# BadgerTechnologies/navigation

Hardware: AMD Instinct MI355X
Metric: scored trajectories/sec (whole node) + costmap inflation cells/sec, 400x400 map (higher is better)
Workload: dtype f64

## Files before the change

navigation_amd/csrc/planner_bfs_rows.hip:

```cpp
#include "planner_bfs_common.h"

namespace navgpu {

#ifdef NAVGPU_BFS_STATS
__device__ unsigned long long g_bfs_stats[16];
#define BFS_STAMP(v) const unsigned long long v = __builtin_amdgcn_s_memtime()
#define BFS_ACC(i, x) bst[i] += (x)
#else
#define BFS_STAMP(v)
#define BFS_ACC(i, x)
#endif
#ifndef NAVGPU_ROWS_RECORD_PAD
#define NAVGPU_ROWS_RECORD_PAD 4
#endif
constexpr uint32_t kRowsRecordPad = NAVGPU_ROWS_RECORD_PAD;
template <int W>
__host__ __device__ inline size_t bfs_rows_lds_words(uint32_t nx, uint32_t ny) {
  constexpr uint32_t Wp = (W + 3) & ~3u;
  const uint32_t nw = bfs_rows_waves(ny);
  return (((size_t)nw * kRowsPerWave * ((nx + 31) >> 5) + 3) & ~(size_t)3) + (size_t)kCareRows * kCareWords + (size_t)(nw + 2) * 2 * kRowsHalo * (2 * Wp + kRowsRecordPad);
}
__device__ __forceinline__ void rowsGroup4(const int g, const uint32_t aw, uint32_t& nz, uint32_t& lo, uint32_t& hi, uint32_t* __restrict__ b,
                                           uint32_t* __restrict__ f, const uint32_t L, const uint32_t R, uint32_t& p) {
  uint32_t u0, u1, u2, u3, t0, t1, t2, t3, st;
  uint64_t c0, c1, c2;
#define NAVGPU_ROWS_DPP " row_mask:0xf bank_mask:0xf bound_ctrl:1\n\t"
  asm volatile(
      "v_mov_b32 %[p], %[f3]\n\t"
      "s_bitcmp1_b32 %[aw], %[g]\n\t"
      "s_cbranch_scc0 1f\n\t"
      "v_alignbit_b32 %[u0], %[f0], %[L], 31\n\t"
      "v_alignbit_b32 %[u1], %[f1], %[f0], 31\n\t"
      "v_alignbit_b32 %[u2], %[f2], %[f1], 31\n\t"
      "v_alignbit_b32 %[u3], %[f3], %[f2], 31\n\t"
      "v_alignbit_b32 %[t0], %[f1], %[f0], 1\n\t"
      "v_alignbit_b32 %[t1], %[f2], %[f1], 1\n\t"
      "v_alignbit_b32 %[t2], %[f3], %[f2], 1\n\t"
      "v_alignbit_b32 %[t3], %[R], %[f3], 1\n\t"
      "v_or_b32_dpp %[u0], %[f0], %[u0] wave_shr:1" NAVGPU_ROWS_DPP
      "v_or_b32_dpp %[u1], %[f1], %[u1] wave_shr:1" NAVGPU_ROWS_DPP
      "v_or_b32_dpp %[u2], %[f2], %[u2] wave_shr:1" NAVGPU_ROWS_DPP
      "v_or_b32_dpp %[u3], %[f3], %[u3] wave_shr:1" NAVGPU_ROWS_DPP
      "v_or_b32_dpp %[t0], %[f0], %[t0] wave_shl:1" NAVGPU_ROWS_DPP
      "v_or_b32_dpp %[t1], %[f1], %[t1] wave_shl:1" NAVGPU_ROWS_DPP
      "v_or_b32_dpp %[t2], %[f2], %[t2] wave_shl:1" NAVGPU_ROWS_DPP
      "v_or_b32_dpp %[t3], %[f3], %[t3] wave_shl:1" NAVGPU_ROWS_DPP
      "v_bitop3_b32 %[f0], %[u0], %[b0], %[t0] bitop3:0x32\n\t"
      "v_bitop3_b32 %[f1], %[u1], %[b1], %[t1] bitop3:0x32\n\t"
      "v_bitop3_b32 %[f2], %[u2], %[b2], %[t2] bitop3:0x32\n\t"
      "v_bitop3_b32 %[f3], %[u3], %[b3], %[t3] bitop3:0x32\n\t"
      "v_or3_b32 %[b0], %[b0], %[u0], %[t0]\n\t"
      "v_or3_b32 %[b1], %[b1], %[u1], %[t1]\n\t"
      "v_or3_b32 %[b2], %[b2], %[u2], %[t2]\n\t"
      "v_or3_b32 %[b3], %[b3], %[u3], %[t3]\n\t"
      "v_or3_b32 %[u0], %[f0], %[f1], %[f2]\n\t"
      "v_cmp_ne_u32_e64 %[c1], 0, %[f0]\n\t"
      "v_or_b32_e32 %[u0], %[u0], %[f3]\n\t"
      "v_cmp_ne_u32_e64 %[c2], 0, %[f3]\n\t"
      "v_cmp_ne_u32_e64 %[c0], 0, %[u0]\n\t"
      "s_cmp_lg_u64 %[c1], 0\n\t"
      "s_cselect_b32 %[st], %[bit], 0\n\t"
      "s_or_b32 %[lo], %[lo], %[st]\n\t"
      "s_cmp_lg_u64 %[c2], 0\n\t"
      "s_cselect_b32 %[st], %[bit], 0\n\t"
      "s_or_b32 %[hi], %[hi], %[st]\n\t"
      "s_cmp_lg_u64 %[c0], 0\n\t"
      "s_cselect_b32 %[st], %[bit], 0\n\t"
      "s_or_b32 %[nz], %[nz], %[st]\n\t"
      "1:\n\t"
      : [b0] "+v"(b[0]), [b1] "+v"(b[1]), [b2] "+v"(b[2]), [b3] "+v"(b[3]), [f0] "+v"(f[0]), [f1] "+v"(f[1]), [f2] "+v"(f[2]), [f3] "+v"(f[3]),
        [p] "=&v"(p), [u0] "=&v"(u0), [u1] "=&v"(u1), [u2] "=&v"(u2), [u3] "=&v"(u3), [t0] "=&v"(t0), [t1] "=&v"(t1), [t2] "=&v"(t2),
        [t3] "=&v"(t3), [nz] "+s"(nz), [lo] "+s"(lo), [hi] "+s"(hi), [c0] "=&s"(c0), [c1] "=&s"(c1), [c2] "=&s"(c2), [st] "=&s"(st)
      : [aw] "s"(aw), [g] "n"(g), [bit] "n"(1 << g), [L] "v"(L), [R] "v"(R)
      : "scc");
#undef NAVGPU_ROWS_DPP
}
template <int W>
__device__ __forceinline__ void bfsRowsGrid(const PlannerDev& pl, const uint32_t inst, const int which, const uint32_t item) {
  constexpr int NG = (W + 3) / 4;
  constexpr int WP = NG * 4;
  constexpr int D = kRowsHalo;
  const BfsRegion rg = bfsRegion(pl, inst);
  const int bx0 = rg.x0, bx1 = rg.x1, by0 = rg.y0, by1 = rg.y1, care_ok = rg.care_ok;
  extern __shared__ __align__(16) uint32_t sm[];
  __shared__ uint32_t s_wave[16];
  __shared__ uint32_t s_flag[3];
  __shared__ uint32_t s_open[3];
  uint32_t tid_ = threadIdx.x, nx_ = pl.nx, ny_ = pl.ny;
  asm volatile("" : "+v"(tid_), "+s"(nx_), "+s"(ny_));
  const uint32_t tid = tid_;
  bfsStamp(pl, tid, item, 0);
  const Geom g = geomOf(pl, inst);
  const uint32_t nx = nx_, ny = ny_, Wr = (nx + 31) >> 5;
  const uint32_t nw = blockDim.x >> 6;
  const uint32_t lane = tid & 63u, wave_id = tid >> 6;
  const int row_i = (int)(wave_id * kRowsPerWave + lane) - D;
  const bool real = row_i >= 0 && row_i < (int)ny;
  const bool owner = real && lane >= (uint32_t)D && lane < 64u - D;
  const uint32_t row = real ? (uint32_t)row_i : 0u;
// ... 27 lines not shown

  uint32_t blocked[WP], fr[WP];
#pragma unroll
  for (int j = 0; j < WP; ++j) {
    blocked[j] = 0xFFFFFFFFu;
    fr[j] = 0;
    if (real && (uint32_t)j < Wr) {
      fr[j] = seedm[row * Wr + j];
      blocked[j] = ~(freew[row * Wr + j] & ((uint32_t)j + 1 == Wr ? last_mask : 0xFFFFFFFFu)) | fr[j];
    }
  }
  const bool wave_in_box = (int)(wave_id * kRowsPerWave) <= by1 && (int)((wave_id + 1) * kRowsPerWave) > by0;
  const bool row_in_box = owner && row_i >= by0 && row_i <= by1;
  const int w0 = rg.w0, w1 = rg.w1;
  const uint32_t region_groups = bfsRegionGroups(rg);
  uint32_t* drow = dist + (size_t)row * nx;
  auto storeCells = [&](int j, uint32_t cells, uint32_t value) { bfsStoreCells(drow + j * 32, cells, value, aligned4); };
  const bool pub_top = lane >= (uint32_t)D && lane < 2u * D, pub_bot = lane >= 64u - 2 * D && lane < 64u - D;
  const uint32_t pub_wr = (((wave_id + 1) * 2 + (pub_top ? 0u : 1u)) * D + (pub_top ? lane - D : lane - (64u - 2 * D))) * RS;
  const bool halo_top = lane < (uint32_t)D, halo_bot = lane >= 64u - D;
  const uint32_t halo_rd = ((halo_top ? (wave_id * 2 + 1) : ((wave_id + 2) * 2)) * D + (halo_top ? lane : lane - (64u - D))) * RS;
  constexpr uint32_t gmask = (1u << NG) - 1u;

  auto activity = [&]() -> uint32_t {
    uint32_t nz = 0, lo = 0, hi = 0;
#pragma unroll
    for (int q = 0; q < NG; ++q) {
      const uint32_t t = fr[4 * q] | fr[4 * q + 1] | fr[4 * q + 2] | fr[4 * q + 3];
      if (__builtin_amdgcn_ballot_w64(t != 0) != 0) {
        nz |= 1u << q;
        if (__builtin_amdgcn_ballot_w64(fr[4 * q] != 0) != 0) lo |= 1u << q;
        if (__builtin_amdgcn_ballot_w64(fr[4 * q + 3] != 0) != 0) hi |= 1u << q;
      }
    }
    return (nz | (lo >> 1) | (hi << 1)) & gmask;
  };
  if (wave_in_box) {
#pragma unroll
    for (int j = 0; j < W; ++j)
      if (j >= w0 && j <= w1 && row_in_box) storeCells(j, fr[j], 0u);
  }
  uint32_t a_own = activity();
  uint32_t level = 0, xch = 0, any_blk = 0;
  bfsStamp(pl, tid, item, 2);
  bool done = false;
#ifdef NAVGPU_BFS_STATS
  unsigned long long bst[9] = {0, 0, 0, 0, 0, 0, 0, 0, 0};
#endif
  while (!done) {
    for (int k = 0; k < D; ++k) {
      BFS_STAMP(ts1);
      BFS_ACC(5, 1);
      const uint32_t aw = __builtin_amdgcn_readfirstlane(a_own);
      BFS_ACC(7, aw != 0 ? 1 : 0);
      BFS_ACC(8, __builtin_popcount(aw));
      if (aw != 0) {
        uint32_t nz = 0, lo = 0, hi = 0;
        uint32_t p[2];
        const uint32_t zero = 0;
#pragma unroll
        for (int q = 0; q < NG; ++q)
          rowsGroup4(q, aw, nz, lo, hi, &blocked[4 * q], &fr[4 * q], q > 0 ? p[(q + 1) & 1] : zero, q + 1 < NG ? fr[q + 1 < NG ? 4 * q + 4 : 0] : zero,
                     p[q & 1]);
        BFS_STAMP(ts2);
        BFS_ACC(1, ts2 - ts1);
        if (wave_in_box && (nz & region_groups) != 0) {
#pragma unroll
          for (int q = 0; q < NG; ++q) {
            if (((nz & region_groups) >> q) & 1u) {
#pragma unroll
              for (int c = 0; c < 4; ++c) {
                const int j = 4 * q + c;
                if (j < W && j >= w0 && j <= w1) {
#ifndef NAVGPU_BFS_X_NOSTORE
                  if (row_in_box && fr[j < W ? j : 0] != 0) storeCells(j, fr[j < W ? j : 0], level + 1);
#endif
                }
              }
            }
          }
        }
        BFS_STAMP(ts3);
        BFS_ACC(2, ts3 - ts2);
        any_blk |= nz;
        a_own = (nz | (lo >> 1) | (hi << 1)) & gmask;
      }
      ++level;
    }
    BFS_STAMP(ts4);
    const uint32_t slot = xch % 3u;
    if (pub_top || pub_bot) {
#pragma unroll
      for (int q = 0; q < WP; q += 4) {
        *reinterpret_cast<uint4*>(edge + pub_wr + q) = make_uint4(fr[q], fr[q + 1], fr[q + 2], fr[q + 3]);
        *reinterpret_cast<uint4*>(edge + pub_wr + WP + q) = make_uint4(blocked[q], blocked[q + 1], blocked[q + 2], blocked[q + 3]);
      }
    }
    if (any_blk) s_flag[slot] = 1;
    if (wave_in_box) {
      uint32_t open_any = 0;
      const uint32_t rr = (uint32_t)(row_i - by0);
#pragma unroll
      for (int j = 0; j < W; ++j) {
        if (j >= w0 && j <= w1) {
          const uint32_t cw_i = (uint32_t)(j - w0);
          if (row_in_box) {
            const uint32_t care = (care_ok != 0 && cw_i < (uint32_t)kCareWords && rr < (uint32_t)kCareRows) ? care_l[rr * kCareWords + cw_i] : (care_ok ? 0u : 0xFFFFFFFFu);
            const int c_lo = max(bx0 - j * 32, 0), c_hi = min(bx1 - j * 32, 31);
            const uint32_t open = (~blocked[j] & care) | fr[j];
            if (c_hi >= c_lo) open_any |= open & (0xFFFFFFFFu >> (31 - c_hi)) & (0xFFFFFFFFu << c_lo);
          }
        }
      }
      if (open_any != 0) s_open[slot] = 1;
    }
    if (tid == 0) {
      s_flag[(xch + 1) % 3u] = 0;
      s_open[(xch + 1) % 3u] = 0;
    }
    BFS_STAMP(ts5);
    BFS_ACC(3, ts5 - ts4);
    __syncthreads();
    done = !s_flag[slot] || !s_open[slot];
    if (!done) {
      if ((halo_top || halo_bot) && real) {
#pragma unroll
        for (int q = 0; q < WP; q += 4) {
          const uint4 v = *reinterpret_cast<const uint4*>(edge + halo_rd + q);
          const uint4 b = *reinterpret_cast<const uint4*>(edge + halo_rd + WP + q);
          fr[q] = v.x;
          fr[q + 1] = v.y;
          fr[q + 2] = v.z;
          fr[q + 3] = v.w;
          blocked[q] = b.x;
          blocked[q + 1] = b.y;
          blocked[q + 2] = b.z;
          blocked[q + 3] = b.w;
        }
      }
      a_own = activity();
      __syncthreads();
    }
    ++xch;
    any_blk = 0;
    BFS_STAMP(ts6);
    BFS_ACC(4, ts6 - ts5);
  }
#ifdef NAVGPU_BFS_STATS
  if (lane == 0)
    for (int k = 0; k < 9; ++k) atomicAdd(&g_bfs_stats[k], bst[k]);
#endif
  bfsStamp(pl, tid, item, 3);

  __syncthreads();
  {
    uint32_t ex[WP], fb[WP];
#pragma unroll
    for (int j = 0; j < WP; ++j) {
      const bool in = owner && (uint32_t)j < Wr;
      fb[j] = in ? (freew[row * Wr + j] & ((uint32_t)j + 1 == Wr ? last_mask : 0xFFFFFFFFu)) : 0u;
      ex[j] = in ? ((blocked[j] & fb[j]) | seedm[row * Wr + j]) : 0u;
    }
    if (pub_top || pub_bot) {
#pragma unroll
      for (int j = 0; j < WP; ++j) edge[pub_wr + j] = ex[j];
    }
    __syncthreads();
// ... 24 lines not shown
__global__ __launch_bounds__(1024, 6) void k_bfs_rows(PlannerDev pl, uint32_t first, uint32_t count, uint32_t* next_item, const uint32_t* order) {
  __shared__ uint32_t s_item;
  const uint32_t total = count * pl.bfs_grids;
  for (;;) {
    if (threadIdx.x == 0) s_item = atomicAdd(next_item, 1u);
    __syncthreads();
    const uint32_t slot = s_item;
    if (slot >= total) break;
    const uint32_t item = order ? order[slot] : slot;
    const uint32_t g = item / count;
    bfsRowsGrid<W>(pl, first + (item - g * count), (int)pl.bfs_grids - 1 - (int)g, item);
    __syncthreads();
  }
}
constexpr int kRows2HaloLanes = 4;
constexpr int kRows2Levels = 2 * kRows2HaloLanes;
constexpr int kRows2PerWave = 2 * (64 - 2 * kRows2HaloLanes);
constexpr int kRows2Words = 32;
__host__ __device__ inline uint32_t bfs_rows2_waves(uint32_t ny) { return (ny + kRows2PerWave - 1) / kRows2PerWave; }
__host__ __device__ inline size_t bfs_rows2_lds_words(uint32_t ny) {
  return (size_t)kCareRows * kCareWords + (size_t)(bfs_rows2_waves(ny) + 2) * 2 * kRows2HaloLanes * 4 * kRows2Words;
}
template <int G>
__device__ __forceinline__ void rows2Group(const uint32_t aw, uint32_t& nz, uint32_t& lo, uint32_t& hi, uint32_t* __restrict__ bA, uint32_t* __restrict__ bB,
                                           uint32_t* __restrict__ fA, uint32_t* __restrict__ fB, uint32_t& pA, uint32_t& pB, const uint32_t rA,
                                           const uint32_t rB) {
  uint32_t u0, u1, u2, u3, v0, v1, v2, v3, h0, h1, h2, h3, st;
#define NAVGPU_ROWS2_HEAD_FIRST                \
  "s_bitcmp1_b32 %[aw], %[g]\n\t"              \
  "s_cbranch_scc0 1f\n\t"                      \
  "v_lshlrev_b32 %[u0], 1, %[fA0]\n\t"         \
  "v_lshlrev_b32 %[v0], 1, %[fB0]\n\t"
#define NAVGPU_ROWS2_HEAD_NEXT                 \
  "s_bitcmp1_b32 %[aw], %[g]\n\t"              \
  "s_cbranch_scc0 1f\n\t"                      \
  "s_bitcmp1_b32 %[aw], %[gp]\n\t"             \
  "s_cbranch_scc1 3f\n\t"                      \
  "v_lshlrev_b32 %[u0], 1, %[fA0]\n\t"         \
  "v_lshlrev_b32 %[v0], 1, %[fB0]\n\t"         \
  "s_branch 4f\n\t"                            \
  "3:\n\t"                                     \
  "v_alignbit_b32 %[u0], %[fA0], %[pA], 31\n\t" \
  "v_alignbit_b32 %[v0], %[fB0], %[pB], 31\n\t" \
  "4:\n\t"
#define NAVGPU_ROWS2_BODY(HEAD)                                                                        \
  asm volatile(                                                                                        \
      HEAD                                                                                             \
      "v_alignbit_b32 %[u1], %[fA1], %[fA0], 31\n\t"                                                   \
      "v_alignbit_b32 %[u2], %[fA2], %[fA1], 31\n\t"                                                   \
      "v_alignbit_b32 %[u3], %[fA3], %[fA2], 31\n\t"                                                   \
// ... 22 lines not shown
      "v_or_b32_dpp %[v1], %[fA1], %[v1] wave_shl:1 row_mask:0xf bank_mask:0xf bound_ctrl:1\n\t"       \
      "v_or_b32_dpp %[v2], %[fA2], %[v2] wave_shl:1 row_mask:0xf bank_mask:0xf bound_ctrl:1\n\t"       \
      "v_or_b32_dpp %[v3], %[fA3], %[v3] wave_shl:1 row_mask:0xf bank_mask:0xf bound_ctrl:1\n\t"       \
      "v_or3_b32 %[v0], %[v0], %[h0], %[fA0]\n\t"                                                      \
      "v_or3_b32 %[v1], %[v1], %[h1], %[fA1]\n\t"                                                      \
      "v_or3_b32 %[v2], %[v2], %[h2], %[fA2]\n\t"                                                      \
      "v_or3_b32 %[v3], %[v3], %[h3], %[fA3]\n\t"                                                      \
      "v_bitop3_b32 %[fA0], %[u0], %[bA0], %[u0] bitop3:0x30\n\t"                                      \
      "v_bitop3_b32 %[fA1], %[u1], %[bA1], %[u1] bitop3:0x30\n\t"                                      \
      "v_bitop3_b32 %[fA2], %[u2], %[bA2], %[u2] bitop3:0x30\n\t"                                      \
      "v_bitop3_b32 %[fA3], %[u3], %[bA3], %[u3] bitop3:0x30\n\t"                                      \
      "v_bitop3_b32 %[fB0], %[v0], %[bB0], %[v0] bitop3:0x30\n\t"                                      \
      "v_bitop3_b32 %[fB1], %[v1], %[bB1], %[v1] bitop3:0x30\n\t"                                      \
      "v_bitop3_b32 %[fB2], %[v2], %[bB2], %[v2] bitop3:0x30\n\t"                                      \
      "v_bitop3_b32 %[fB3], %[v3], %[bB3], %[v3] bitop3:0x30\n\t"                                      \
      "v_or_b32_e32 %[bA0], %[bA0], %[u0]\n\t"                                                         \
      "v_or_b32_e32 %[bA1], %[bA1], %[u1]\n\t"                                                         \
      "v_or_b32_e32 %[bA2], %[bA2], %[u2]\n\t"                                                         \
      "v_or_b32_e32 %[bA3], %[bA3], %[u3]\n\t"                                                         \
      "v_or_b32_e32 %[bB0], %[bB0], %[v0]\n\t"                                                         \
      "v_or_b32_e32 %[bB1], %[bB1], %[v1]\n\t"                                                         \
      "v_or_b32_e32 %[bB2], %[bB2], %[v2]\n\t"                                                         \
      "v_or_b32_e32 %[bB3], %[bB3], %[v3]\n\t"                                                         \
      "v_or_b32_e32 %[h0], %[fA0], %[fB0]\n\t"                                                         \
      "v_or_b32_e32 %[h3], %[fA3], %[fB3]\n\t"                                                         \
      "v_or3_b32 %[h1], %[fA1], %[fA2], %[fB1]\n\t"                                                    \
      "v_or3_b32 %[h2], %[h0], %[h3], %[fB2]\n\t"                                                      \
      "v_or_b32_e32 %[h1], %[h1], %[h2]\n\t"                                                           \
      "v_cmp_ne_u32_e32 vcc, 0, %[h1]\n\t"                                                             \
      "s_cbranch_vccz 1f\n\t"                                                                          \
      "s_bitset1_b32 %[nz], %[g]\n\t"                                                                  \
      "v_cmp_ne_u32_e32 vcc, 0, %[h0]\n\t"                                                             \
      "s_cbranch_vccz 3f\n\t"                                                                          \
      "s_bitset1_b32 %[lo], %[g]\n\t"                                                                  \
      "3:\n\t"                                                                                         \
      "v_cmp_ne_u32_e32 vcc, 0, %[h3]\n\t"                                                             \
      "s_cbranch_vccz 1f\n\t"                                                                          \
      "s_bitset1_b32 %[hi], %[g]\n\t"                                                                  \
      "1:\n\t"                                                                                         \
      : [bA0] "+v"(bA[0]), [bA1] "+v"(bA[1]), [bA2] "+v"(bA[2]), [bA3] "+v"(bA[3]), [bB0] "+v"(bB[0]), [bB1] "+v"(bB[1]), [bB2] "+v"(bB[2]),  \
        [bB3] "+v"(bB[3]), [fA0] "+v"(fA[0]), [fA1] "+v"(fA[1]), [fA2] "+v"(fA[2]), [fA3] "+v"(fA[3]), [fB0] "+v"(fB[0]), [fB1] "+v"(fB[1]),   \
        [fB2] "+v"(fB[2]), [fB3] "+v"(fB[3]), [pA] "+v"(pA), [pB] "+v"(pB), [nz] "+s"(nz), [lo] "+s"(lo), [hi] "+s"(hi), [u0] "=&v"(u0),       \
        [u1] "=&v"(u1), [u2] "=&v"(u2), [u3] "=&v"(u3), [v0] "=&v"(v0), [v1] "=&v"(v1), [v2] "=&v"(v2), [v3] "=&v"(v3), [h0] "=&v"(h0),        \
        [h1] "=&v"(h1), [h2] "=&v"(h2), [h3] "=&v"(h3), [st] "=&s"(st)                                                                         \
      : [aw] "s"(aw), [g] "n"(G), [gp] "n"(G > 0 ? G - 1 : 0), [rA] "v"(rA), [rB] "v"(rB)                                                      \
      : "vcc", "scc")
  if constexpr (G == 0) NAVGPU_ROWS2_BODY(NAVGPU_ROWS2_HEAD_FIRST);
  else NAVGPU_ROWS2_BODY(NAVGPU_ROWS2_HEAD_NEXT);
#undef NAVGPU_ROWS2_BODY
#undef NAVGPU_ROWS2_HEAD_FIRST
#undef NAVGPU_ROWS2_HEAD_NEXT
}
template <int G>
__device__ __forceinline__ void rows2Level(const uint32_t aw, uint32_t& nz, uint32_t& lo, uint32_t& hi, uint32_t* __restrict__ blA, uint32_t* __restrict__ blB,
                                           uint32_t* __restrict__ frA, uint32_t* __restrict__ frB, uint32_t& pA, uint32_t& pB, const uint32_t zero) {
  constexpr int NG = kRows2Words / 4;
  if constexpr (G < NG) {
    rows2Group<G>(aw, nz, lo, hi, blA + 4 * G, blB + 4 * G, frA + 4 * G, frB + 4 * G, pA, pB, G + 1 < NG ? frA[G + 1 < NG ? 4 * G + 4 : 0] : zero,
                  G + 1 < NG ? frB[G + 1 < NG ? 4 * G + 4 : 0] : zero);
    rows2Level<G + 1>(aw, nz, lo, hi, blA, blB, frA, frB, pA, pB, zero);
  }
}
__device__ __forceinline__ void bfsRows2Grid(const PlannerDev& pl, const uint32_t inst, const int which, const uint32_t item, uint32_t* seedw) {
  constexpr int W = kRows2Words, NG = W / 4, D = kRows2Levels, HL = kRows2HaloLanes;
  const BfsRegion rg = bfsRegion(pl, inst);
  const int bx0 = rg.x0, bx1 = rg.x1, by0 = rg.y0, by1 = rg.y1, care_ok = rg.care_ok;
  extern __shared__ __align__(16) uint32_t sm[];
  __shared__ uint32_t s_wave[16];
  __shared__ uint32_t s_flag[3];
  __shared__ uint32_t s_open[3];
  uint32_t tid_ = threadIdx.x, nx_ = pl.nx, ny_ = pl.ny;
  asm volatile("" : "+v"(tid_), "+s"(nx_), "+s"(ny_));
  const uint32_t tid = tid_;
  bfsStamp(pl, tid, item, 0);
  const Geom g = geomOf(pl, inst);
  const uint32_t nx = nx_, ny = ny_, Wr = (nx + 31) >> 5;
  const uint32_t nw = blockDim.x >> 6;
  const uint32_t lane = tid & 63u, wave_id = tid >> 6;
  const int rowA_i = (int)(wave_id * kRows2PerWave) + 2 * ((int)lane - HL), rowB_i = rowA_i + 1;
  const bool own_lane = lane >= (uint32_t)HL && lane < 64u - HL;
  const bool realA = rowA_i >= 0 && rowA_i < (int)ny, realB = rowB_i >= 0 && rowB_i < (int)ny;
  const bool ownerA = realA && own_lane, ownerB = realB && own_lane;
  const uint32_t rowA = realA ? (uint32_t)rowA_i : 0u, rowB = realB ? (uint32_t)rowB_i : 0u;
// ... 47 lines not shown
#pragma unroll
    for (int c = 0; c < 4; ++c) {
      const int j = 4 * q + c;
      const bool in = (uint32_t)j < Wr;
      asm volatile("v_mov_b32 %0, %1" : "=v"(frA[j]) : "v"(sa[c]));
      asm volatile("v_mov_b32 %0, %1" : "=v"(frB[j]) : "v"(sb[c]));
      blA[j] = (in && realA) ? (~(fa[c] & colMask(j)) | sa[c]) : 0xFFFFFFFFu;
      blB[j] = (in && realB) ? (~(fb[c] & colMask(j)) | sb[c]) : 0xFFFFFFFFu;
    }
  }
  const bool wave_in_box = (int)(wave_id * kRows2PerWave) <= by1 && (int)((wave_id + 1) * kRows2PerWave) > by0;
  const bool inA = ownerA && rowA_i >= by0 && rowA_i <= by1, inB = ownerB && rowB_i >= by0 && rowB_i <= by1;
  const int w0 = rg.w0, w1 = rg.w1;
  const uint32_t region_groups = bfsRegionGroups(rg);
  auto storeCells = [&](const uint32_t row, int j, uint32_t cells, uint32_t value) {
    bfsStoreCells(dist + (size_t)row * nx + j * 32, cells, value, aligned4);
  };
  const bool pub_top = lane >= (uint32_t)HL && lane < 2u * HL, pub_bot = lane >= 64u - 2 * HL && lane < 64u - HL;
  const uint32_t pub_wr = (((wave_id + 1) * 2 + (pub_top ? 0u : 1u)) * HL + (pub_top ? lane - HL : lane - (64u - 2 * HL))) * 4 * W;
  const bool halo_top = lane < (uint32_t)HL, halo_bot = lane >= 64u - HL;
  const uint32_t halo_rd = ((halo_top ? (wave_id * 2 + 1) : ((wave_id + 2) * 2)) * HL + (halo_top ? lane : lane - (64u - HL))) * 4 * W;
  constexpr uint32_t gmask = (1u << NG) - 1u;

  auto activity = [&]() -> uint32_t {
    uint32_t nz = 0, lo = 0, hi = 0;
#pragma unroll
    for (int q = 0; q < NG; ++q) {
      const uint32_t t = frA[4 * q] | frA[4 * q + 1] | frA[4 * q + 2] | frA[4 * q + 3] | frB[4 * q] | frB[4 * q + 1] | frB[4 * q + 2] | frB[4 * q + 3];
      if (__builtin_amdgcn_ballot_w64(t != 0) != 0) {
        nz |= 1u << q;
        if (__builtin_amdgcn_ballot_w64((frA[4 * q] | frB[4 * q]) != 0) != 0) lo |= 1u << q;
        if (__builtin_amdgcn_ballot_w64((frA[4 * q + 3] | frB[4 * q + 3]) != 0) != 0) hi |= 1u << q;
      }
    }
    return (nz | (lo >> 1) | (hi << 1)) & gmask;
  };
  if (wave_in_box) {
#pragma unroll
    for (int j = 0; j < W; ++j)
      if (j >= w0 && j <= w1) {
        if (inA) storeCells(rowA, j, frA[j], 0u);
        if (inB) storeCells(rowB, j, frB[j], 0u);
      }
  }
  uint32_t a_own = activity();
  uint32_t level = 0, xch = 0, any_blk = 0;
  bfsStamp(pl, tid, item, 2);
  bool done = false;
#ifdef NAVGPU_BFS_STATS
  unsigned long long bst[9] = {0, 0, 0, 0, 0, 0, 0, 0, 0};
#endif
  while (!done) {
    for (int k = 0; k < D; ++k) {
      BFS_STAMP(ts1);
      BFS_ACC(5, 1);
      const uint32_t aw = __builtin_amdgcn_readfirstlane(a_own);
      BFS_ACC(7, aw != 0 ? 1 : 0);
      BFS_ACC(8, __builtin_popcount(aw));
      if (aw != 0) {
        uint32_t nz = 0, lo = 0, hi = 0;
        uint32_t pA = 0, pB = 0;
        const uint32_t zero = 0;
        rows2Level<0>(aw, nz, lo, hi, blA, blB, frA, frB, pA, pB, zero);
        BFS_STAMP(ts2);
        BFS_ACC(1, ts2 - ts1);
        if (wave_in_box && (nz & region_groups) != 0) {
#pragma unroll
          for (int q = 0; q < NG; ++q) {
            if (((nz & region_groups) >> q) & 1u) {
#pragma unroll
              for (int c = 0; c < 4; ++c) {
                const int j = 4 * q + c;
                if (j >= w0 && j <= w1) {
                  if (inA && frA[j] != 0) storeCells(rowA, j, frA[j], level + 1);
                  if (inB && frB[j] != 0) storeCells(rowB, j, frB[j], level + 1);
                }
              }
            }
          }
        }
        BFS_STAMP(ts3);
        BFS_ACC(2, ts3 - ts2);
        any_blk |= nz;
        a_own = (nz | (lo >> 1) | (hi << 1)) & gmask;
      }
      ++level;
    }
    BFS_STAMP(ts4);
    const uint32_t slot = xch % 3u;
    auto quad = [&](const uint32_t* w4) {
      uint32_t a, b, c, d;
      asm volatile("v_mov_b32 %0, %4\n\tv_mov_b32 %1, %5\n\tv_mov_b32 %2, %6\n\tv_mov_b32 %3, %7" : "=&v"(a), "=&v"(b), "=&v"(c), "=&v"(d) : "v"(w4[0]), "v"(w4[1]), "v"(w4[2]), "v"(w4[3]));
      return make_uint4(a, b, c, d);
    };
    auto unquad = [&](const uint4 v, uint32_t* w4) {
      asm volatile("v_mov_b32 %0, %4\n\tv_mov_b32 %1, %5\n\tv_mov_b32 %2, %6\n\tv_mov_b32 %3, %7" : "=&v"(w4[0]), "=&v"(w4[1]), "=&v"(w4[2]), "=&v"(w4[3]) : "v"(v.x), "v"(v.y), "v"(v.z), "v"(v.w));
    };
    if (pub_top || pub_bot) {
#pragma unroll
      for (int q = 0; q < W; q += 4) {
        *reinterpret_cast<uint4*>(edge + pub_wr + q) = quad(frA + q);
        *reinterpret_cast<uint4*>(edge + pub_wr + W + q) = quad(blA + q);
        *reinterpret_cast<uint4*>(edge + pub_wr + 2 * W + q) = quad(frB + q);
        *reinterpret_cast<uint4*>(edge + pub_wr + 3 * W + q) = quad(blB + q);
      }
    }
    if (any_blk) s_flag[slot] = 1;
    if (wave_in_box) {
      uint32_t open_any = 0;
      const uint32_t rrA = (uint32_t)(rowA_i - by0), rrB = (uint32_t)(rowB_i - by0);
#pragma unroll
      for (int j = 0; j < W; ++j) {
        if (j >= w0 && j <= w1) {
          const uint32_t cw_i = (uint32_t)(j - w0);
          const uint32_t cm = bfsColMask(bx0, bx1, j);
          if (inA) {
            const uint32_t care = (care_ok != 0 && cw_i < (uint32_t)kCareWords && rrA < (uint32_t)kCareRows) ? care_l[rrA * kCareWords + cw_i] : (care_ok ? 0u : 0xFFFFFFFFu);
            open_any |= ((~blA[j] & care) | frA[j]) & cm;
          }
          if (inB) {
            const uint32_t care = (care_ok != 0 && cw_i < (uint32_t)kCareWords && rrB < (uint32_t)kCareRows) ? care_l[rrB * kCareWords + cw_i] : (care_ok ? 0u : 0xFFFFFFFFu);
            open_any |= ((~blB[j] & care) | frB[j]) & cm;
          }
        }
      }
      if (open_any != 0) s_open[slot] = 1;
    }
    if (tid == 0) {
      s_flag[(xch + 1) % 3u] = 0;
      s_open[(xch + 1) % 3u] = 0;
    }
    BFS_STAMP(ts5);
    BFS_ACC(3, ts5 - ts4);
    __syncthreads();
    done = !s_flag[slot] || !s_open[slot];
    if (!done) {
      if (halo_top || halo_bot) {
#pragma unroll
        for (int q = 0; q < W; q += 4) {
          if (realA) {
            unquad(*reinterpret_cast<const uint4*>(edge + halo_rd + q), frA + q);
            unquad(*reinterpret_cast<const uint4*>(edge + halo_rd + W + q), blA + q);
          }
          if (realB) {
            unquad(*reinterpret_cast<const uint4*>(edge + halo_rd + 2 * W + q), frB + q);
            unquad(*reinterpret_cast<const uint4*>(edge + halo_rd + 3 * W + q), blB + q);
          }
        }
      }
      a_own = activity();
      __syncthreads();
    }
    ++xch;
    any_blk = 0;
    BFS_STAMP(ts6);
    BFS_ACC(4, ts6 - ts5);
  }
#ifdef NAVGPU_BFS_STATS
  if (lane == 0)
    for (int k = 0; k < 9; ++k) atomicAdd(&g_bfs_stats[k], bst[k]);
#endif
  bfsStamp(pl, tid, item, 3);

  __syncthreads();
  {
#pragma unroll
    for (int q = 0; q < NG; ++q) {
      const uint4 sA = ownerA ? rowWords(seedw, rowA, q) : make_uint4(0, 0, 0, 0), sB = ownerB ? rowWords(seedw, rowB, q) : make_uint4(0, 0, 0, 0);
      const uint4 fA = ownerA ? rowWords(freew, rowA, q) : make_uint4(0, 0, 0, 0), fB = ownerB ? rowWords(freew, rowB, q) : make_uint4(0, 0, 0, 0);
      const uint32_t sa[4] = {sA.x, sA.y, sA.z, sA.w}, sb[4] = {sB.x, sB.y, sB.z, sB.w}, fa[4] = {fA.x, fA.y, fA.z, fA.w}, fb[4] = {fB.x, fB.y, fB.z, fB.w};
#pragma unroll
      for (int c = 0; c < 4; ++c) {
        const int j = 4 * q + c;
        const bool in = (uint32_t)j < Wr;
        blA[j] = (in && ownerA) ? ((blA[j] & fa[c] & colMask(j)) | sa[c]) : 0u;
        blB[j] = (in && ownerB) ? ((blB[j] & fb[c] & colMask(j)) | sb[c]) : 0u;
      }
// ... 107 lines not shown
```

Baseline: 5.645 billion.

## Fix active word groups per halo round and drop per-level activity bookkeeping

The bitset BFS kernels now compute the active word-group mask once per halo exchange round, not after every level. The mask is widened so a group counts as neighbouring-active only when frontier bits lie within D bits of the group edge, because that is as far as a frontier can spread in D levels. Inside the round each level now just ORs a nonzero flag into a 64-bit scalar accumulator, replacing the lo/hi/nz scalar compare-select chains and vcc branches. The trade-off is that groups which go idle mid-round are still processed until the next exchange. The W==20 specialisation keeps the old per-level path.

Result: faster. 6.054 billion, median of 6 (+7.2%).

```diff
diff --git a/navigation_amd/csrc/planner_bfs_rows.hip b/navigation_amd/csrc/planner_bfs_rows.hip
--- a/navigation_amd/csrc/planner_bfs_rows.hip
+++ b/navigation_amd/csrc/planner_bfs_rows.hip
@@ -20,61 +20,80 @@
   const uint32_t nw = bfs_rows_waves(ny);
   return (((size_t)nw * kRowsPerWave * ((nx + 31) >> 5) + 3) & ~(size_t)3) + (size_t)kCareRows * kCareWords + (size_t)(nw + 2) * 2 * kRowsHalo * (2 * Wp + kRowsRecordPad);
 }
-__device__ __forceinline__ void rowsGroup4(const int g, const uint32_t aw, uint32_t& nz, uint32_t& lo, uint32_t& hi, uint32_t* __restrict__ b,
-                                           uint32_t* __restrict__ f, const uint32_t L, const uint32_t R, uint32_t& p) {
+#define NAVGPU_ROWS_DPP " row_mask:0xf bank_mask:0xf bound_ctrl:1\n\t"
+#define NAVGPU_ROWS_GROUP_WORDS                                    \
+  "v_mov_b32 %[p], %[f3]\n\t"                                      \
+  "s_bitcmp1_b32 %[aw], %[g]\n\t"                                  \
+  "s_cbranch_scc0 1f\n\t"                                          \
+  "v_alignbit_b32 %[u0], %[f0], %[L], 31\n\t"                      \
+  "v_alignbit_b32 %[u1], %[f1], %[f0], 31\n\t"                     \
+  "v_alignbit_b32 %[u2], %[f2], %[f1], 31\n\t"                     \
+  "v_alignbit_b32 %[u3], %[f3], %[f2], 31\n\t"                     \
+  "v_alignbit_b32 %[t0], %[f1], %[f0], 1\n\t"                      \
+  "v_alignbit_b32 %[t1], %[f2], %[f1], 1\n\t"                      \
+  "v_alignbit_b32 %[t2], %[f3], %[f2], 1\n\t"                      \
+  "v_alignbit_b32 %[t3], %[R], %[f3], 1\n\t"                       \
+  "v_or_b32_dpp %[u0], %[f0], %[u0] wave_shr:1" NAVGPU_ROWS_DPP    \
+  "v_or_b32_dpp %[u1], %[f1], %[u1] wave_shr:1" NAVGPU_ROWS_DPP    \
+  "v_or_b32_dpp %[u2], %[f2], %[u2] wave_shr:1" NAVGPU_ROWS_DPP    \
+  "v_or_b32_dpp %[u3], %[f3], %[u3] wave_shr:1" NAVGPU_ROWS_DPP    \
+  "v_or_b32_dpp %[t0], %[f0], %[t0] wave_shl:1" NAVGPU_ROWS_DPP    \
+  "v_or_b32_dpp %[t1], %[f1], %[t1] wave_shl:1" NAVGPU_ROWS_DPP    \
+  "v_or_b32_dpp %[t2], %[f2], %[t2] wave_shl:1" NAVGPU_ROWS_DPP    \
+  "v_or_b32_dpp %[t3], %[f3], %[t3] wave_shl:1" NAVGPU_ROWS_DPP    \
+  "v_bitop3_b32 %[f0], %[u0], %[b0], %[t0] bitop3:0x32\n\t"        \
+  "v_bitop3_b32 %[f1], %[u1], %[b1], %[t1] bitop3:0x32\n\t"        \
+  "v_bitop3_b32 %[f2], %[u2], %[b2], %[t2] bitop3:0x32\n\t"        \
+  "v_bitop3_b32 %[f3], %[u3], %[b3], %[t3] bitop3:0x32\n\t"        \
+  "v_or3_b32 %[b0], %[b0], %[u0], %[t0]\n\t"                       \
+  "v_or3_b32 %[b1], %[b1], %[u1], %[t1]\n\t"                       \
+  "v_or3_b32 %[b2], %[b2], %[u2], %[t2]\n\t"                       \
+  "v_or3_b32 %[b3], %[b3], %[u3], %[t3]\n\t"
+#define NAVGPU_ROWS_GROUP_REGS                                                                                                              \
+  [b0] "+v"(b[0]), [b1] "+v"(b[1]), [b2] "+v"(b[2]), [b3] "+v"(b[3]), [f0] "+v"(f[0]), [f1] "+v"(f[1]), [f2] "+v"(f[2]), [f3] "+v"(f[3]), \
+      [p] "=&v"(p), [u0] "=&v"(u0), [u1] "=&v"(u1), [u2] "=&v"(u2), [u3] "=&v"(u3), [t0] "=&v"(t0), [t1] "=&v"(t1), [t2] "=&v"(t2),       \
+      [t3] "=&v"(t3)
+__device__ __forceinline__ void rowsGroup4(const int g, const uint32_t aw, uint64_t& acc, uint32_t* __restrict__ b, uint32_t* __restrict__ f,
+                                           const uint32_t L, const uint32_t R, uint32_t& p) {
+  uint32_t u0, u1, u2, u3, t0, t1, t2, t3;
+  uint64_t c0;
+  asm volatile(NAVGPU_ROWS_GROUP_WORDS
+               "v_or3_b32 %[u0], %[f0], %[f1], %[f2]\n\t"
+               "v_or_b32_e32 %[u0], %[u0], %[f3]\n\t"
+               "v_cmp_ne_u32_e64 %[c0], 0, %[u0]\n\t"
+               "s_or_b64 %[acc], %[acc], %[c0]\n\t"
+               "1:\n\t"
+               : NAVGPU_ROWS_GROUP_REGS, [acc] "+s"(acc), [c0] "=&s"(c0)
+               : [aw] "s"(aw), [g] "n"(g), [L] "v"(L), [R] "v"(R)
+               : "scc");
+}
+__device__ __forceinline__ void rowsGroup4PerLevel(const int g, const uint32_t aw, uint32_t& nz, uint32_t& lo, uint32_t& hi, uint32_t* __restrict__ b,
+                                                   uint32_t* __restrict__ f, const uint32_t L, const uint32_t R, uint32_t& p) {
   uint32_t u0, u1, u2, u3, t0, t1, t2, t3, st;
   uint64_t c0, c1, c2;
-#define NAVGPU_ROWS_DPP " row_mask:0xf bank_mask:0xf bound_ctrl:1\n\t"
-  asm volatile(
-      "v_mov_b32 %[p], %[f3]\n\t"
-      "s_bitcmp1_b32 %[aw], %[g]\n\t"
-      "s_cbranch_scc0 1f\n\t"
-      "v_alignbit_b32 %[u0], %[f0], %[L], 31\n\t"
-      "v_alignbit_b32 %[u1], %[f1], %[f0], 31\n\t"
-      "v_alignbit_b32 %[u2], %[f2], %[f1], 31\n\t"
-      "v_alignbit_b32 %[u3], %[f3], %[f2], 31\n\t"
-      "v_alignbit_b32 %[t0], %[f1], %[f0], 1\n\t"
-      "v_alignbit_b32 %[t1], %[f2], %[f1], 1\n\t"
-      "v_alignbit_b32 %[t2], %[f3], %[f2], 1\n\t"
-      "v_alignbit_b32 %[t3], %[R], %[f3], 1\n\t"
-      "v_or_b32_dpp %[u0], %[f0], %[u0] wave_shr:1" NAVGPU_ROWS_DPP
-      "v_or_b32_dpp %[u1], %[f1], %[u1] wave_shr:1" NAVGPU_ROWS_DPP
-      "v_or_b32_dpp %[u2], %[f2], %[u2] wave_shr:1" NAVGPU_ROWS_DPP
-      "v_or_b32_dpp %[u3], %[f3], %[u3] wave_shr:1" NAVGPU_ROWS_DPP
-      "v_or_b32_dpp %[t0], %[f0], %[t0] wave_shl:1" NAVGPU_ROWS_DPP
-      "v_or_b32_dpp %[t1], %[f1], %[t1] wave_shl:1" NAVGPU_ROWS_DPP
-      "v_or_b32_dpp %[t2], %[f2], %[t2] wave_shl:1" NAVGPU_ROWS_DPP
-      "v_or_b32_dpp %[t3], %[f3], %[t3] wave_shl:1" NAVGPU_ROWS_DPP
-      "v_bitop3_b32 %[f0], %[u0], %[b0], %[t0] bitop3:0x32\n\t"
-      "v_bitop3_b32 %[f1], %[u1], %[b1], %[t1] bitop3:0x32\n\t"
-      "v_bitop3_b32 %[f2], %[u2], %[b2], %[t2] bitop3:0x32\n\t"
-      "v_bitop3_b32 %[f3], %[u3], %[b3], %[t3] bitop3:0x32\n\t"
-      "v_or3_b32 %[b0], %[b0], %[u0], %[t0]\n\t"
-      "v_or3_b32 %[b1], %[b1], %[u1], %[t1]\n\t"
-      "v_or3_b32 %[b2], %[b2], %[u2], %[t2]\n\t"
-      "v_or3_b32 %[b3], %[b3], %[u3], %[t3]\n\t"
-      "v_or3_b32 %[u0], %[f0], %[f1], %[f2]\n\t"
-      "v_cmp_ne_u32_e64 %[c1], 0, %[f0]\n\t"
-      "v_or_b32_e32 %[u0], %[u0], %[f3]\n\t"
-      "v_cmp_ne_u32_e64 %[c2], 0, %[f3]\n\t"
-      "v_cmp_ne_u32_e64 %[c0], 0, %[u0]\n\t"
-      "s_cmp_lg_u64 %[c1], 0\n\t"
-      "s_cselect_b32 %[st], %[bit], 0\n\t"
-      "s_or_b32 %[lo], %[lo], %[st]\n\t"
-      "s_cmp_lg_u64 %[c2], 0\n\t"
-      "s_cselect_b32 %[st], %[bit], 0\n\t"
-      "s_or_b32 %[hi], %[hi], %[st]\n\t"
-      "s_cmp_lg_u64 %[c0], 0\n\t"
-      "s_cselect_b32 %[st], %[bit], 0\n\t"
-      "s_or_b32 %[nz], %[nz], %[st]\n\t"
-      "1:\n\t"
-      : [b0] "+v"(b[0]), [b1] "+v"(b[1]), [b2] "+v"(b[2]), [b3] "+v"(b[3]), [f0] "+v"(f[0]), [f1] "+v"(f[1]), [f2] "+v"(f[2]), [f3] "+v"(f[3]),
-        [p] "=&v"(p), [u0] "=&v"(u0), [u1] "=&v"(u1), [u2] "=&v"(u2), [u3] "=&v"(u3), [t0] "=&v"(t0), [t1] "=&v"(t1), [t2] "=&v"(t2),
-        [t3] "=&v"(t3), [nz] "+s"(nz), [lo] "+s"(lo), [hi] "+s"(hi), [c0] "=&s"(c0), [c1] "=&s"(c1), [c2] "=&s"(c2), [st] "=&s"(st)
-      : [aw] "s"(aw), [g] "n"(g), [bit] "n"(1 << g), [L] "v"(L), [R] "v"(R)
-      : "scc");
+  asm volatile(NAVGPU_ROWS_GROUP_WORDS
+               "v_or3_b32 %[u0], %[f0], %[f1], %[f2]\n\t"
+               "v_cmp_ne_u32_e64 %[c1], 0, %[f0]\n\t"
+               "v_or_b32_e32 %[u0], %[u0], %[f3]\n\t"
+               "v_cmp_ne_u32_e64 %[c2], 0, %[f3]\n\t"
+               "v_cmp_ne_u32_e64 %[c0], 0, %[u0]\n\t"
+               "s_cmp_lg_u64 %[c1], 0\n\t"
+               "s_cselect_b32 %[st], %[bit], 0\n\t"
+               "s_or_b32 %[lo], %[lo], %[st]\n\t"
+               "s_cmp_lg_u64 %[c2], 0\n\t"
+               "s_cselect_b32 %[st], %[bit], 0\n\t"
+               "s_or_b32 %[hi], %[hi], %[st]\n\t"
+               "s_cmp_lg_u64 %[c0], 0\n\t"
+               "s_cselect_b32 %[st], %[bit], 0\n\t"
+               "s_or_b32 %[nz], %[nz], %[st]\n\t"
+               "1:\n\t"
+               : NAVGPU_ROWS_GROUP_REGS, [nz] "+s"(nz), [lo] "+s"(lo), [hi] "+s"(hi), [c0] "=&s"(c0), [c1] "=&s"(c1), [c2] "=&s"(c2), [st] "=&s"(st)
+               : [aw] "s"(aw), [g] "n"(g), [bit] "n"(1 << g), [L] "v"(L), [R] "v"(R)
+               : "scc");
+}
+#undef NAVGPU_ROWS_GROUP_REGS
+#undef NAVGPU_ROWS_GROUP_WORDS
 #undef NAVGPU_ROWS_DPP
-}
 template <int W>
 __device__ __forceinline__ void bfsRowsGrid(const PlannerDev& pl, const uint32_t inst, const int which, const uint32_t item) {
   constexpr int NG = (W + 3) / 4;
@@ -148,6 +167,9 @@
   const uint32_t halo_rd = ((halo_top ? (wave_id * 2 + 1) : ((wave_id + 2) * 2)) * D + (halo_top ? lane : lane - (64u - D))) * RS;
   constexpr uint32_t gmask = (1u << NG) - 1u;
 
+  constexpr bool kBlockLive = W != 20;
+  static_assert(D >= 1 && D < 32, "the edge masks take D bits of one word");
+  constexpr uint32_t edge_lo = kBlockLive ? (1u << D) - 1u : 0xFFFFFFFFu, edge_hi = kBlockLive ? ~(0xFFFFFFFFu >> D) : 0xFFFFFFFFu;
   auto activity = [&]() -> uint32_t {
     uint32_t nz = 0, lo = 0, hi = 0;
 #pragma unroll
@@ -155,8 +177,8 @@
       const uint32_t t = fr[4 * q] | fr[4 * q + 1] | fr[4 * q + 2] | fr[4 * q + 3];
       if (__builtin_amdgcn_ballot_w64(t != 0) != 0) {
         nz |= 1u << q;
-        if (__builtin_amdgcn_ballot_w64(fr[4 * q] != 0) != 0) lo |= 1u << q;
-        if (__builtin_amdgcn_ballot_w64(fr[4 * q + 3] != 0) != 0) hi |= 1u << q;
+        if (__builtin_amdgcn_ballot_w64((fr[4 * q] & edge_lo) != 0) != 0) lo |= 1u << q;
+        if (__builtin_amdgcn_ballot_w64((fr[4 * q + 3] & edge_hi) != 0) != 0) hi |= 1u << q;
       }
     }
     return (nz | (lo >> 1) | (hi << 1)) & gmask;
@@ -167,51 +189,87 @@
       if (j >= w0 && j <= w1 && row_in_box) storeCells(j, fr[j], 0u);
   }
   uint32_t a_own = activity();
-  uint32_t level = 0, xch = 0, any_blk = 0;
+  uint32_t level = 0, xch = 0;
   bfsStamp(pl, tid, item, 2);
   bool done = false;
 #ifdef NAVGPU_BFS_STATS
   unsigned long long bst[9] = {0, 0, 0, 0, 0, 0, 0, 0, 0};
 #endif
+  auto storeNew = [&](const uint32_t groups) {
+    if (wave_in_box && (groups & region_groups) != 0) {
+#pragma unroll
+      for (int q = 0; q < NG; ++q) {
+        if (((groups & region_groups) >> q) & 1u) {
+#pragma unroll
+          for (int c = 0; c < 4; ++c) {
+            const int j = 4 * q + c;
+            if (j < W && j >= w0 && j <= w1) {
+#ifndef NAVGPU_BFS_X_NOSTORE
+              if (row_in_box && fr[j < W ? j : 0] != 0) storeCells(j, fr[j < W ? j : 0], level + 1);
+#endif
+            }
+          }
+        }
+      }
+    }
+  };
   while (!done) {
-    for (int k = 0; k < D; ++k) {
-      BFS_STAMP(ts1);
-      BFS_ACC(5, 1);
+    bool any_new;
+    if constexpr (kBlockLive) {
       const uint32_t aw = __builtin_amdgcn_readfirstlane(a_own);
-      BFS_ACC(7, aw != 0 ? 1 : 0);
-      BFS_ACC(8, __builtin_popcount(aw));
-      if (aw != 0) {
-        uint32_t nz = 0, lo = 0, hi = 0;
-        uint32_t p[2];
-        const uint32_t zero = 0;
-#pragma unroll
-        for (int q = 0; q < NG; ++q)
-          rowsGroup4(q, aw, nz, lo, hi, &blocked[4 * q], &fr[4 * q], q > 0 ? p[(q + 1) & 1] : zero, q + 1 < NG ? fr[q + 1 < NG ? 4 * q + 4 : 0] : zero,
-                     p[q & 1]);
-        BFS_STAMP(ts2);
-        BFS_ACC(1, ts2 - ts1);
-        if (wave_in_box && (nz & region_groups) != 0) {
-#pragma unroll
-          for (int q = 0; q < NG; ++q) {
-            if (((nz & region_groups) >> q) & 1u) {
-#pragma unroll
-              for (int c = 0; c < 4; ++c) {
-                const int j = 4 * q + c;
-                if (j < W && j >= w0 && j <= w1) {
-#ifndef NAVGPU_BFS_X_NOSTORE
-                  if (row_in_box && fr[j < W ? j : 0] != 0) storeCells(j, fr[j < W ? j : 0], level + 1);
-#endif
-                }
-              }
-            }
-          }
-        }
-        BFS_STAMP(ts3);
-        BFS_ACC(2, ts3 - ts2);
-        any_blk |= nz;
-        a_own = (nz | (lo >> 1) | (hi << 1)) & gmask;
-      }
-      ++level;
+      uint64_t acc = 0;
+      if (aw == 0) {
+        BFS_ACC(5, D);
+        level += D;
+      } else {
+        for (int k = 0; k < D; ++k) {
+          BFS_STAMP(ts1);
+          BFS_ACC(5, 1);
+          BFS_ACC(7, 1);
+          BFS_ACC(8, __builtin_popcount(aw));
+          uint32_t awk = aw;
+          asm volatile("" : "+s"(awk));
+          uint32_t p[2];
+          const uint32_t zero = 0;
+#pragma unroll
+          for (int q = 0; q < NG; ++q)
+            rowsGroup4(q, awk, acc, &blocked[4 * q], &fr[4 * q], q > 0 ? p[(q + 1) & 1] : zero, q + 1 < NG ? fr[q + 1 < NG ? 4 * q + 4 : 0] : zero, p[q & 1]);
+          BFS_STAMP(ts2);
+          BFS_ACC(1, ts2 - ts1);
+          storeNew(awk);
+          BFS_STAMP(ts3);
+          BFS_ACC(2, ts3 - ts2);
+          ++level;
+        }
+      }
+      any_new = acc != 0;
+    } else {
+      uint32_t any_blk = 0;
+      for (int k = 0; k < D; ++k) {
+        BFS_STAMP(ts1);
+        BFS_ACC(5, 1);
+        const uint32_t aw = __builtin_amdgcn_readfirstlane(a_own);
+        BFS_ACC(7, aw != 0 ? 1 : 0);
+        BFS_ACC(8, __builtin_popcount(aw));
+        if (aw != 0) {
+          uint32_t nz = 0, lo = 0, hi = 0;
+          uint32_t p[2];
+          const uint32_t zero = 0;
+#pragma unroll
+          for (int q = 0; q < NG; ++q)
+            rowsGroup4PerLevel(q, aw, nz, lo, hi, &blocked[4 * q], &fr[4 * q], q > 0 ? p[(q + 1) & 1] : zero, q + 1 < NG ? fr[q + 1 < NG ? 4 * q + 4 : 0] : zero,
+                               p[q & 1]);
+          BFS_STAMP(ts2);
+          BFS_ACC(1, ts2 - ts1);
+          storeNew(nz);
+          BFS_STAMP(ts3);
+          BFS_ACC(2, ts3 - ts2);
+          any_blk |= nz;
+          a_own = (nz | (lo >> 1) | (hi << 1)) & gmask;
+        }
+        ++level;
+      }
+      any_new = any_blk != 0;
     }
     BFS_STAMP(ts4);
     const uint32_t slot = xch % 3u;
@@ -222,7 +280,7 @@
         *reinterpret_cast<uint4*>(edge + pub_wr + WP + q) = make_uint4(blocked[q], blocked[q + 1], blocked[q + 2], blocked[q + 3]);
       }
     }
-    if (any_blk) s_flag[slot] = 1;
+    if (any_new) s_flag[slot] = 1;
     if (wave_in_box) {
       uint32_t open_any = 0;
       const uint32_t rr = (uint32_t)(row_i - by0);
@@ -268,7 +326,6 @@
       __syncthreads();
     }
     ++xch;
-    any_blk = 0;
     BFS_STAMP(ts6);
     BFS_ACC(4, ts6 - ts5);
   }
@@ -339,10 +396,10 @@
   return (size_t)kCareRows * kCareWords + (size_t)(bfs_rows2_waves(ny) + 2) * 2 * kRows2HaloLanes * 4 * kRows2Words;
 }
 template <int G>
-__device__ __forceinline__ void rows2Group(const uint32_t aw, uint32_t& nz, uint32_t& lo, uint32_t& hi, uint32_t* __restrict__ bA, uint32_t* __restrict__ bB,
-                                           uint32_t* __restrict__ fA, uint32_t* __restrict__ fB, uint32_t& pA, uint32_t& pB, const uint32_t rA,
-                                           const uint32_t rB) {
-  uint32_t u0, u1, u2, u3, v0, v1, v2, v3, h0, h1, h2, h3, st;
+__device__ __forceinline__ void rows2Group(const uint32_t aw, uint64_t& acc, uint32_t* __restrict__ bA, uint32_t* __restrict__ bB, uint32_t* __restrict__ fA,
+                                           uint32_t* __restrict__ fB, uint32_t& pA, uint32_t& pB, const uint32_t rA, const uint32_t rB) {
+  uint32_t u0, u1, u2, u3, v0, v1, v2, v3, h0, h1, h2, h3;
+  uint64_t c0;
 #define NAVGPU_ROWS2_HEAD_FIRST                \
   "s_bitcmp1_b32 %[aw], %[g]\n\t"              \
   "s_cbranch_scc0 1f\n\t"                      \
@@ -411,29 +468,20 @@
       "v_or_b32_e32 %[bB1], %[bB1], %[v1]\n\t"                                                         \
       "v_or_b32_e32 %[bB2], %[bB2], %[v2]\n\t"                                                         \
       "v_or_b32_e32 %[bB3], %[bB3], %[v3]\n\t"                                                         \
-      "v_or_b32_e32 %[h0], %[fA0], %[fB0]\n\t"                                                         \
-      "v_or_b32_e32 %[h3], %[fA3], %[fB3]\n\t"                                                         \
-      "v_or3_b32 %[h1], %[fA1], %[fA2], %[fB1]\n\t"                                                    \
-      "v_or3_b32 %[h2], %[h0], %[h3], %[fB2]\n\t"                                                      \
-      "v_or_b32_e32 %[h1], %[h1], %[h2]\n\t"                                                           \
-      "v_cmp_ne_u32_e32 vcc, 0, %[h1]\n\t"                                                             \
-      "s_cbranch_vccz 1f\n\t"                                                                          \
-      "s_bitset1_b32 %[nz], %[g]\n\t"                                                                  \
-      "v_cmp_ne_u32_e32 vcc, 0, %[h0]\n\t"                                                             \
-      "s_cbranch_vccz 3f\n\t"                                                                          \
-      "s_bitset1_b32 %[lo], %[g]\n\t"                                                                  \
-      "3:\n\t"                                                                                         \
-      "v_cmp_ne_u32_e32 vcc, 0, %[h3]\n\t"                                                             \
-      "s_cbranch_vccz 1f\n\t"                                                                          \
-      "s_bitset1_b32 %[hi], %[g]\n\t"                                                                  \
+      "v_or3_b32 %[h0], %[fA0], %[fB0], %[fA1]\n\t"                                                    \
+      "v_or3_b32 %[h1], %[fB1], %[fA2], %[fB2]\n\t"                                                    \
+      "v_or3_b32 %[h0], %[h0], %[fA3], %[fB3]\n\t"                                                     \
+      "v_or_b32_e32 %[h0], %[h0], %[h1]\n\t"                                                           \
+      "v_cmp_ne_u32_e64 %[c0], 0, %[h0]\n\t"                                                           \
+      "s_or_b64 %[acc], %[acc], %[c0]\n\t"                                                             \
       "1:\n\t"                                                                                         \
       : [bA0] "+v"(bA[0]), [bA1] "+v"(bA[1]), [bA2] "+v"(bA[2]), [bA3] "+v"(bA[3]), [bB0] "+v"(bB[0]), [bB1] "+v"(bB[1]), [bB2] "+v"(bB[2]),  \
         [bB3] "+v"(bB[3]), [fA0] "+v"(fA[0]), [fA1] "+v"(fA[1]), [fA2] "+v"(fA[2]), [fA3] "+v"(fA[3]), [fB0] "+v"(fB[0]), [fB1] "+v"(fB[1]),   \
-        [fB2] "+v"(fB[2]), [fB3] "+v"(fB[3]), [pA] "+v"(pA), [pB] "+v"(pB), [nz] "+s"(nz), [lo] "+s"(lo), [hi] "+s"(hi), [u0] "=&v"(u0),       \
+        [fB2] "+v"(fB[2]), [fB3] "+v"(fB[3]), [pA] "+v"(pA), [pB] "+v"(pB), [acc] "+s"(acc), [c0] "=&s"(c0), [u0] "=&v"(u0),                  \
         [u1] "=&v"(u1), [u2] "=&v"(u2), [u3] "=&v"(u3), [v0] "=&v"(v0), [v1] "=&v"(v1), [v2] "=&v"(v2), [v3] "=&v"(v3), [h0] "=&v"(h0),        \
-        [h1] "=&v"(h1), [h2] "=&v"(h2), [h3] "=&v"(h3), [st] "=&s"(st)                                                                         \
+        [h1] "=&v"(h1), [h2] "=&v"(h2), [h3] "=&v"(h3)                                                                                         \
       : [aw] "s"(aw), [g] "n"(G), [gp] "n"(G > 0 ? G - 1 : 0), [rA] "v"(rA), [rB] "v"(rB)                                                      \
-      : "vcc", "scc")
+      : "scc")
   if constexpr (G == 0) NAVGPU_ROWS2_BODY(NAVGPU_ROWS2_HEAD_FIRST);
   else NAVGPU_ROWS2_BODY(NAVGPU_ROWS2_HEAD_NEXT);
 #undef NAVGPU_ROWS2_BODY
@@ -441,13 +489,13 @@
 #undef NAVGPU_ROWS2_HEAD_NEXT
 }
 template <int G>
-__device__ __forceinline__ void rows2Level(const uint32_t aw, uint32_t& nz, uint32_t& lo, uint32_t& hi, uint32_t* __restrict__ blA, uint32_t* __restrict__ blB,
-                                           uint32_t* __restrict__ frA, uint32_t* __restrict__ frB, uint32_t& pA, uint32_t& pB, const uint32_t zero) {
+__device__ __forceinline__ void rows2Level(const uint32_t aw, uint64_t& acc, uint32_t* __restrict__ blA, uint32_t* __restrict__ blB, uint32_t* __restrict__ frA,
+                                           uint32_t* __restrict__ frB, uint32_t& pA, uint32_t& pB, const uint32_t zero) {
   constexpr int NG = kRows2Words / 4;
   if constexpr (G < NG) {
-    rows2Group<G>(aw, nz, lo, hi, blA + 4 * G, blB + 4 * G, frA + 4 * G, frB + 4 * G, pA, pB, G + 1 < NG ? frA[G + 1 < NG ? 4 * G + 4 : 0] : zero,
+    rows2Group<G>(aw, acc, blA + 4 * G, blB + 4 * G, frA + 4 * G, frB + 4 * G, pA, pB, G + 1 < NG ? frA[G + 1 < NG ? 4 * G + 4 : 0] : zero,
                   G + 1 < NG ? frB[G + 1 < NG ? 4 * G + 4 : 0] : zero);
-    rows2Level<G + 1>(aw, nz, lo, hi, blA, blB, frA, frB, pA, pB, zero);
+    rows2Level<G + 1>(aw, acc, blA, blB, frA, frB, pA, pB, zero);
   }
 }
 __device__ __forceinline__ void bfsRows2Grid(const PlannerDev& pl, const uint32_t inst, const int which, const uint32_t item, uint32_t* seedw) {
@@ -541,6 +589,8 @@
   const uint32_t halo_rd = ((halo_top ? (wave_id * 2 + 1) : ((wave_id + 2) * 2)) * HL + (halo_top ? lane : lane - (64u - HL))) * 4 * W;
   constexpr uint32_t gmask = (1u << NG) - 1u;
 
+  static_assert(D >= 1 && D < 32, "the edge masks take D bits of one word");
+  constexpr uint32_t edge_lo = (1u << D) - 1u, edge_hi = ~(0xFFFFFFFFu >> D);
   auto activity = [&]() -> uint32_t {
     uint32_t nz = 0, lo = 0, hi = 0;
 #pragma unroll
@@ -548,8 +598,8 @@
       const uint32_t t = frA[4 * q] | frA[4 * q + 1] | frA[4 * q + 2] | frA[4 * q + 3] | frB[4 * q] | frB[4 * q + 1] | frB[4 * q + 2] | frB[4 * q + 3];
       if (__builtin_amdgcn_ballot_w64(t != 0) != 0) {
         nz |= 1u << q;
-        if (__builtin_amdgcn_ballot_w64((frA[4 * q] | frB[4 * q]) != 0) != 0) lo |= 1u << q;
-        if (__builtin_amdgcn_ballot_w64((frA[4 * q + 3] | frB[4 * q + 3]) != 0) != 0) hi |= 1u << q;
+        if (__builtin_amdgcn_ballot_w64(((frA[4 * q] | frB[4 * q]) & edge_lo) != 0) != 0) lo |= 1u << q;
+        if (__builtin_amdgcn_ballot_w64(((frA[4 * q + 3] | frB[4 * q + 3]) & edge_hi) != 0) != 0) hi |= 1u << q;
       }
     }
     return (nz | (lo >> 1) | (hi << 1)) & gmask;
@@ -563,46 +613,48 @@
       }
   }
   uint32_t a_own = activity();
-  uint32_t level = 0, xch = 0, any_blk = 0;
+  uint32_t level = 0, xch = 0;
   bfsStamp(pl, tid, item, 2);
   bool done = false;
 #ifdef NAVGPU_BFS_STATS
   unsigned long long bst[9] = {0, 0, 0, 0, 0, 0, 0, 0, 0};
 #endif
   while (!done) {
+    const uint32_t aw = __builtin_amdgcn_readfirstlane(a_own);
+    uint64_t acc = 0;
     for (int k = 0; k < D; ++k) {
       BFS_STAMP(ts1);
       BFS_ACC(5, 1);
-      const uint32_t aw = __builtin_amdgcn_readfirstlane(a_own);
-      BFS_ACC(7, aw != 0 ? 1 : 0);
-      BFS_ACC(8, __builtin_popcount(aw));
-      if (aw != 0) {
-        uint32_t nz = 0, lo = 0, hi = 0;
-        uint32_t pA = 0, pB = 0;
-        const uint32_t zero = 0;
-        rows2Level<0>(aw, nz, lo, hi, blA, blB, frA, frB, pA, pB, zero);
-        BFS_STAMP(ts2);
-        BFS_ACC(1, ts2 - ts1);
-        if (wave_in_box && (nz & region_groups) != 0) {
-#pragma unroll
-          for (int q = 0; q < NG; ++q) {
-            if (((nz & region_groups) >> q) & 1u) {
-#pragma unroll
-              for (int c = 0; c < 4; ++c) {
-                const int j = 4 * q + c;
-                if (j >= w0 && j <= w1) {
-                  if (inA && frA[j] != 0) storeCells(rowA, j, frA[j], level + 1);
-                  if (inB && frB[j] != 0) storeCells(rowB, j, frB[j], level + 1);
-                }
+      uint32_t awk = aw;
+      asm volatile("" : "+s"(awk));
+      BFS_ACC(7, awk != 0 ? 1 : 0);
+      BFS_ACC(8, __builtin_popcount(awk));
+      if (awk == 0) {
+        ++level;
+        continue;
+      }
+      uint32_t pA = 0, pB = 0;
+      const uint32_t zero = 0;
+      rows2Level<0>(awk, acc, blA, blB, frA, frB, pA, pB, zero);
+      BFS_STAMP(ts2);
+      BFS_ACC(1, ts2 - ts1);
+      if (wave_in_box && (awk & region_groups) != 0) {
+#pragma unroll
+        for (int q = 0; q < NG; ++q) {
+          if (((awk & region_groups) >> q) & 1u) {
+#pragma unroll
+            for (int c = 0; c < 4; ++c) {
+              const int j = 4 * q + c;
+              if (j >= w0 && j <= w1) {
+                if (inA && frA[j] != 0) storeCells(rowA, j, frA[j], level + 1);
+                if (inB && frB[j] != 0) storeCells(rowB, j, frB[j], level + 1);
               }
             }
           }
         }
-        BFS_STAMP(ts3);
-        BFS_ACC(2, ts3 - ts2);
-        any_blk |= nz;
-        a_own = (nz | (lo >> 1) | (hi << 1)) & gmask;
-      }
+      }
+      BFS_STAMP(ts3);
+      BFS_ACC(2, ts3 - ts2);
       ++level;
     }
     BFS_STAMP(ts4);
@@ -624,7 +676,7 @@
         *reinterpret_cast<uint4*>(edge + pub_wr + 3 * W + q) = quad(blB + q);
       }
     }
-    if (any_blk) s_flag[slot] = 1;
+    if (acc != 0) s_flag[slot] = 1;
     if (wave_in_box) {
       uint32_t open_any = 0;
       const uint32_t rrA = (uint32_t)(rowA_i - by0), rrB = (uint32_t)(rowB_i - by0);
@@ -671,7 +723,6 @@
       __syncthreads();
     }
     ++xch;
-    any_blk = 0;
     BFS_STAMP(ts6);
     BFS_ACC(4, ts6 - ts5);
   }
```
